# gabrielspmoreira/chameleon_recsys

Hardware: NVIDIA H100
Metric: NAR train interactions/sec (higher is better)
Workload: dtype f32 (wgmma: bf16x3 (error-compensated) forward, single-pass TF32 backward; fp32 accumulate)

## Files before the change

chameleon_recsys_b200/_lib.py:

```python
from __future__ import annotations

import ctypes as C
import os
from typing import Optional

HERE = os.path.dirname(os.path.abspath(__file__))
LIB_PATH = os.path.join(HERE, 'libnar_b200.so')

NAR_MAX_SEGMENTS = 24
NAR_MAX_SRC = 16
NAR_MAX_COLS = 1024

ACT_NONE, ACT_LEAKY, ACT_TANH = 0, 1, 2


class NarError(RuntimeError):
    pass


class Segment(C.Structure):
    _fields_ = [('kind', C.c_int32), ('col', C.c_int32), ('width', C.c_int32), ('card', C.c_int32),
                ('src', C.c_int32), ('ld', C.c_int32), ('table', C.c_void_p), ('grad', C.c_void_p)]


# ... 41 lines not shown
class StepIO(C.Structure):
    _fields_ = [('B', C.c_int64), ('Bg', C.c_int64), ('T', C.c_int64), ('sess0', C.c_int64), ('L', C.c_int64),
                ('L_global', C.c_int64), ('L_cap', C.c_int64), ('global_step', C.c_int64),
                ('sampler_step', C.c_uint32), ('train', C.c_int32),
                ('all_items', C.c_void_p), ('event_ts', C.c_void_p), ('item_clicked', C.c_void_p), ('label_next', C.c_void_p),
                ('buffer', C.c_void_p), ('max_ts', C.c_void_p), ('pop_norm', C.c_void_p),
                ('ctx_int', C.c_void_p * NAR_MAX_SRC), ('ctx_float', C.c_void_p * NAR_MAX_SRC),
                ('pos_idx', C.c_void_p), ('sess_off', C.c_void_p),
                ('prep_ws', C.c_void_p), ('prep_ws_bytes', C.c_int64), ('ws', C.c_void_p), ('ws_bytes', C.c_int64),
                ('loss', C.c_void_p)]


class NoveltyReg(C.Structure):
    _fields_ = [('factor', C.c_float), ('log_base', C.c_float), ('pop_norm', C.c_void_p), ('cand_ids', C.c_void_p),
                ('loss_nov', C.c_void_p)]


class GemmEpilogue(C.Structure):
    _fields_ = [('bias', C.c_void_p), ('act', C.c_int32), ('dact', C.c_int32), ('aux', C.c_void_p),
                ('ld_aux', C.c_int64), ('accumulate', C.c_int32), ('split_k', C.c_int32),
                ('precision', C.c_int32), ('b_lo', C.c_void_p), ('b_bf16', C.c_void_p), ('ld_bf16', C.c_int64),
                ('a_scale', C.c_void_p), ('ld_a_scale', C.c_int64), ('a_scale_group', C.c_int64),
                ('pred', C.c_void_p), ('d_pred', C.c_void_p), ('ld_pred', C.c_int64), ('pred_group', C.c_int64),
                ('car_pp', C.c_void_p), ('car_pc', C.c_void_p), ('car_pi', C.c_void_p), ('car_pos_idx', C.c_void_p),
                ('car_neg_uidx', C.c_void_p), ('car_dpp', C.c_void_p), ('car_dpc', C.c_void_p), ('car_dpi', C.c_void_p),
                ('ld_car', C.c_int64), ('car_k', C.c_int64)]


_lib: Optional[C.CDLL] = None

i64, i32, f32, vp, u64, u32 = C.c_int64, C.c_int32, C.c_float, C.c_void_p, C.c_uint64, C.c_uint32

_SIGNATURES = {
    'nar_abi_version': (C.c_int, []),
    'nar_abi_struct_size': (C.c_int, [C.c_int]),
    'nar_status_string': (C.c_char_p, [C.c_int]),
    'nar_ctx_create': (C.c_int, [C.c_int, C.POINTER(vp)]),
    'nar_ctx_destroy': (C.c_int, [vp]),
    'nar_gather_features': (C.c_int, [vp, C.POINTER(FeaturePlanC), vp, vp, C.POINTER(RowLayout), vp, vp, vp, vp]),
    'nar_gather_features_bwd': (C.c_int, [vp, C.POINTER(FeaturePlanC), vp, vp, C.POINTER(RowLayout), vp, vp, vp, vp, vp, vp]),
    'nar_build_base_rows': (C.c_int, [vp, i64, vp, vp, vp, vp, i64, vp, i64, vp, vp, vp]),
    'nar_sample_negatives_uidx': (C.c_int, [vp, vp, i64, i64, i64, i64, vp, i64, i64, i64, u64, u32, vp, vp,
                                            C.POINTER(vp), C.POINTER(vp), vp, i64, vp]),
    'nar_car_combine': (C.c_int, [vp, vp, vp, vp, vp, i64, i64, i64, C.c_int, vp, vp]),
    'nar_car_combine_t': (C.c_int, [vp, vp, vp, vp, vp, i64, i64, i64, C.c_int, vp, i64, vp]),
    'nar_engine_create': (C.c_int, [vp, C.POINTER(ModelCfg), C.POINTER(vp)]),
    'nar_engine_destroy': (C.c_int, [vp]),
# ... 114 lines not shown
```

chameleon_recsys_b200/csrc/engine.cu:

```cuda
#include "common.cuh"
#include <string.h>
#include <stdio.h>
#include <stdlib.h>

extern "C" int nar_sample_negatives_uidx(nar_ctx*, const int64_t*, int64_t, int64_t, int64_t, int64_t, const int64_t*, int64_t,
                                         int64_t, int64_t, uint64_t, uint32_t, int64_t*, int32_t*, const int64_t**,
                                         const int32_t**, void*, int64_t, void*);
namespace nar {
int recommend_rows(const int32_t* pos_idx, int64_t L, const int64_t* item_clicked, const int64_t* cand_ids, int64_t N,
                   int32_t* row_pos, int64_t* row_item, cudaStream_t st);
}

namespace {

constexpr int N_EVENTS = 64;

inline int64_t align_up(int64_t x, int64_t a) { return (x + a - 1) / a * a; }

struct Carver {
  char* base; int64_t off;
  explicit Carver(void* b) : base(static_cast<char*>(b)), off(0) {}
  template <typename T> T* take(int64_t n) {
    T* p = base ? reinterpret_cast<T*>(base + off) : nullptr;
    off = align_up(off + (n > 0 ? n : 1) * (int64_t)sizeof(T), 256);
// ... 178 lines not shown
    chk(nar_gemm_tf32(e->ctx, M, N, Kd, X, ldx, x_kmajor, W(off_W), ldw, 0, Y, ldy, &ep, st));
  }
  void dgrad(const float* dY, int64_t lddy, int64_t off_W, int64_t ldw, float* dX, int64_t lddx, int64_t M, int64_t n_in,
             int64_t n_out, int dact, const float* auxp, int64_t ld_aux, int accumulate, cudaStream_t st) {
    nar_gemm_epilogue ep; memset(&ep, 0, sizeof(ep));
    ep.dact = dact; ep.aux = auxp; ep.ld_aux = ld_aux; ep.accumulate = accumulate; ep.split_k = accumulate ? 0 : 1;
    ep.precision = c.bwd_precision;
    chk(nar_gemm_tf32(e->ctx, M, n_in, n_out, dY, lddy, 1, W(off_W), ldw, 1, dX, lddx, &ep, st));
  }
  void wgrad(const float* X, int64_t ldx, const float* dY, int64_t lddy, int64_t off_W, int64_t ldw, int64_t n_in, int64_t n_out,
             int64_t rows, cudaStream_t st, const float* a_scale = nullptr, int64_t ld_scale = 0, int64_t group = 0) {
    nar_gemm_epilogue ep; memset(&ep, 0, sizeof(ep));
    ep.a_scale = a_scale; ep.ld_a_scale = ld_scale; ep.a_scale_group = group;
    ep.accumulate = 1; ep.split_k = 0; ep.precision = c.bwd_precision;
    chk(nar_gemm_tf32(e->ctx, n_in, n_out, rows, X, ldx, 0, dY, lddy, 0, G(off_W), ldw, &ep, st));
  }
  void wgrad_xt(const float* XT, int64_t ldxt, const float* dY, int64_t lddy, int64_t off_W, int64_t ldw, int64_t n_in,
                int64_t n_out, int64_t rows, cudaStream_t st) {
    nar_gemm_epilogue ep; memset(&ep, 0, sizeof(ep));
    ep.accumulate = 1; ep.split_k = 0; ep.precision = c.bwd_precision;
    chk(nar_gemm_tf32_dt(e->ctx, n_out, n_in, rows, dY, lddy, 0, XT, ldxt, 1, G(off_W), ldw, &ep, st));
  }
  void dgrad_prod(const float* dY, int64_t lddy, int64_t off_W, int64_t ldw, const float* cand, const float* pred, int64_t group,
                  float* dX, float* dpred, int64_t M, int64_t n_in, int64_t n_out, cudaStream_t st) {
    nar_gemm_epilogue ep; memset(&ep, 0, sizeof(ep));
    ep.dact = NAR_ACT_TANH; ep.aux = cand; ep.ld_aux = n_in; ep.split_k = 1; ep.precision = c.bwd_precision;
    ep.pred = pred; ep.d_pred = dpred; ep.ld_pred = n_in; ep.pred_group = group;
    chk(nar_gemm_tf32(e->ctx, M, n_in, n_out, dY, lddy, 1, W(off_W), ldw, 1, dX, n_in, &ep, st));
  }
  void dgrad_car(const float* dY, int64_t lddy, int64_t off_W, int64_t ldw, const float* PP, const float* PC, const float* PI,
                 const int32_t* pos_idx, const int32_t* neg_uidx, float* dPP, float* dPC, float* dPI, int64_t M, int64_t n_in,
                 int64_t n_out, cudaStream_t st) {
    nar_gemm_epilogue ep; memset(&ep, 0, sizeof(ep));
    ep.dact = NAR_ACT_LEAKY_RELU; ep.split_k = 1; ep.precision = c.bwd_precision;
    ep.car_pp = PP; ep.car_pc = PC; ep.car_pi = PI; ep.car_pos_idx = pos_idx; ep.car_neg_uidx = neg_uidx;
    ep.car_dpp = dPP; ep.car_dpc = dPC; ep.car_dpi = dPI; ep.ld_car = n_in; ep.car_k = c.K;
    chk(nar_gemm_tf32(e->ctx, M, n_in, n_out, dY, lddy, 1, W(off_W), ldw, 1, nullptr, 0, &ep, st));
  }
  void bgrad(const float* dY, int64_t ld, int64_t rows, int64_t cols, int64_t off_b, cudaStream_t st) {
    chk(nar_colsum_add(dY, rows, cols, ld, G(off_b), st));
  }
  void dropout(const float* src, float* dst, int64_t rows, int64_t cols, const int32_t* row_pos, int tensor_id, cudaStream_t st) {
    chk(nar_dropout_rows(src, dst, rows, cols, cols, row_pos, io->L, c.K + 1, c.K, tensor_id, c.keep_prob, c.dropout_seed,
                         (uint32_t)(io->global_step + 1), st));
  }
  void scorer(const float* Ec, const float* PR, int64_t n_pos, int64_t n_cand, bool fused, float* PD, float* Z1, float* Z2,
              float* Z3, float* logits, float* loss, float inv_count, float* dZ3, float* dE, float* dPR,
              const nar_novelty_reg* nov) {
    const int64_t R = n_pos * n_cand, C = c.C;
    if (c.ranking == 0) {
// ... 84 lines not shown
  nar_novelty_reg nov; memset(&nov, 0, sizeof(nov));
  nov.factor = c.novelty_reg_factor; nov.log_base = c.plan.log_base_novelty; nov.pop_norm = io->pop_norm;
  nov.cand_ids = pb.row_item + L; nov.loss_nov = io->loss + 2;
  const nar_novelty_reg* novp = c.novelty_reg_factor > 0.f ? &nov : nullptr;
  const bool fused = fused_product(e);
  s.scorer(Ec, sb.PR, L, n_cand, fused, sb.PD, sb.Z1, sb.Z2, sb.Z3, sb.logits, io->loss, inv_count, train ? sb.dZ3 : nullptr,
           train ? sb.dE + L * C : nullptr, train ? sb.dPR : nullptr, novp);
  if (c.reg_l2 > 0.f && c.rank == 0) { cudaStream_t st = s.fork(); s.chk(nar_l2_loss_add(c.params, c.reg_end, c.reg_l2, io->loss + 1, st)); }
  if (!train || s.rc) { s.join(); return s.rc; }

  float* dEc = sb.dE + L * C;
  if (c.ranking == 0) {
    { cudaStream_t st = s.fork(); s.wgrad(sb.Z2, 64, sb.dZ3, 32, c.off_M[2], c.ld_M[2], 64, 32, Rc, st); s.bgrad(sb.dZ3, 32, Rc, 32, c.off_c[2], st); }
    s.dgrad(sb.dZ3, 32, c.off_M[2], c.ld_M[2], sb.dZ2, 64, Rc, 64, 32, NAR_ACT_LEAKY_RELU, sb.Z2, 64, 0, main);
    { cudaStream_t st = s.fork(); s.wgrad(sb.Z1, 128, sb.dZ2, 64, c.off_M[1], c.ld_M[1], 128, 64, Rc, st); s.bgrad(sb.dZ2, 64, Rc, 64, c.off_c[1], st); }
    s.dgrad(sb.dZ2, 64, c.off_M[1], c.ld_M[1], sb.dZ1, 128, Rc, 128, 64, NAR_ACT_LEAKY_RELU, sb.Z1, 128, 0, main);
    {
      cudaStream_t st = s.fork();
      if (fused) s.wgrad(Ec, C, sb.dZ1, 128, c.off_M[0], c.ld_M[0], C, 128, Rc, st, sb.PR, C, n_cand);
      else s.wgrad(sb.PD, C, sb.dZ1, 128, c.off_M[0], c.ld_M[0], C, 128, Rc, st);
      s.bgrad(sb.dZ1, 128, Rc, 128, c.off_c[0], st);
    }
    if (fused) {
      s.dgrad_prod(sb.dZ1, 128, c.off_M[0], c.ld_M[0], Ec, sb.PR, n_cand, dEc, sb.dPR, Rc, C, 128, main);
    } else {
      s.dgrad(sb.dZ1, 128, c.off_M[0], c.ld_M[0], sb.dPD, C, Rc, C, 128, NAR_ACT_NONE, nullptr, 0, 0, main);
      s.chk(nar_mul_pred_bwd(sb.dPD, Ec, sb.PR, L, n_cand, C, NAR_ACT_TANH, dEc, sb.dPR, main));
    }
  } else {
    s.chk(nar_act_bwd(dEc, Ec, Rc * C, NAR_ACT_TANH, dEc, main));
  }
  {
    cudaStream_t st = s.fork();
    if (c.dedup) s.wgrad_xt(sb.H1cT, sb.ldr, dEc, C, c.off_W2, C, C, C, Rc, st);
    else s.wgrad(H1c, C, dEc, C, c.off_W2, C, C, C, Rc, st);
    s.bgrad(dEc, C, Rc, C, c.off_b2, st);
  }
  {
    s.chk(nar_act_bwd(sb.dPR, sb.PR, L * C, NAR_ACT_TANH, sb.dPR, main));
    { cudaStream_t st = s.fork(); s.wgrad(sb.F1, 512, sb.dPR, C, c.off_W4, C, 512, C, L, st); s.bgrad(sb.dPR, C, L, C, c.off_b4, st); }
    s.dgrad(sb.dPR, C, c.off_W4, C, sb.dF1, 512, L, 512, C, NAR_ACT_LEAKY_RELU, sb.F1, 512, 0, main);
    if (drop) s.dropout(sb.dF1, sb.dF1, L, 512, io->pos_idx, 4, main);
    const float* rnn_out = drop ? sb.HOd[c.layers - 1] : sb.HO[c.layers - 1];
    { cudaStream_t st = s.fork(); s.wgrad(rnn_out, Hp, sb.dF1, 512, c.off_W3, 512, Hp, 512, L, st); s.bgrad(sb.dF1, 512, L, 512, c.off_b3, st); }
    s.dgrad(sb.dF1, 512, c.off_W3, 512, sb.dHO, Hp, L, Hp, 512, NAR_ACT_NONE, nullptr, 0, 0, main);
    float* dho = sb.dHO;
    for (int i = c.layers - 1; i >= 0; --i) {
      if (drop) s.dropout(dho, dho, L, Hp, io->pos_idx, 8 + i, main);
      const float* x_in = i == 0 ? sb.E : (drop ? sb.HOd[i - 1] : sb.HO[i - 1]);
      const int64_t n_in = i == 0 ? C : Hp;
      const int64_t gw = gate_blocks(c) * Hp;
      if (c.rnn_cell == NAR_CELL_GRU) {
        float* cand_T = e->WhT[i] + 2 * Hp * Hp;
        s.chk(nar_transpose_f32(s.W(c.off_Wh[i]), Hp, 2 * Hp, 2 * Hp, e->WhT[i], Hp, main));
        s.chk(nar_transpose_f32(s.W(c.off_Whc[i]), Hp, Hp, Hp, cand_T, Hp, main));
        s.chk(nar_gru_bwd(e->ctx, dho, sb.HO[i], sb.GT[i], sb.UO[i], sb.CD[i], e->WhT[i], cand_T, io->sess_off, B, Hp, sb.dGX[i],
                          sb.HPV[i], main));
      } else {
        s.chk(nar_transpose_f32(s.W(c.off_Wh[i]), Hp, gw, gw, e->WhT[i], Hp, main));
// ... 327 lines not shown
                                    void* stream) {
  if (!e || !io || !io->ws || !q_pos || !cand_ids || !out_ids || !io->buffer || !io->pop_norm || !io->item_clicked) return NAR_ERR_INVALID;
  if (io->train) return NAR_ERR_INVALID;
  return run_recommend(e, io, q_rows, q_pos, Q, cand_ids, N, top_n, exclude_session_clicks, q_block, n_block, out_ids, out_scores,
                       out_probs, as_stream(stream));
}

extern "C" int64_t nar_engine_launch_count(const nar_engine* e) { return e ? e->launches : 0; }

extern "C" int nar_engine_buffer(const nar_engine* e, const nar_step_io* io, const char* name, void** ptr, int64_t* rows, int64_t* ld) {
  if (!e || !io || !name || !ptr) return NAR_ERR_INVALID;
  const nar_model_cfg& c = e->cfg;
  const int64_t L = io->L, K = c.K, n_cand = K + 1, Rc = L * n_cand, R = L + Rc;
  PrepBufs pb; StepBufs sb;
  prep_carve(e, io->Bg, io->B, io->T, io->L_cap, io->prep_ws, &pb);
  step_carve(e, io->L_cap, io->train, io->ws, &sb);
  const int64_t NB = 2 * L + pb.U;
  struct Ent { const char* n; void* p; int64_t r, l; };
  const Ent tab[] = {
      {"neg", pb.neg, io->Bg * io->T, K}, {"neg_uidx", pb.neg_uidx, io->Bg * io->T, K}, {"stats", pb.stats, 1, 24},
      {"row_pos", pb.row_pos, R, 1}, {"row_item", pb.row_item, R, 1}, {"base_pos", pb.base_pos, NB, 1},
      {"base_item", pb.base_item, NB, 1},
      {"X", sb.X, c.dedup ? NB : R, c.Fp}, {"dX", sb.dX, c.dedup ? NB : R, c.Fp}, {"H1", sb.H1, R, c.C}, {"H1cT", sb.H1cT, c.C, sb.ldr}, {"E", sb.E, R, c.C},
      {"dE", sb.dE, R, c.C}, {"dH1", sb.dH1, R, c.C}, {"F1", sb.F1, L, 512}, {"PR", sb.PR, L, c.C},
      {"logits", sb.logits, L, n_cand}, {"PD", sb.PD, Rc, c.C}, {"Z1", sb.Z1, Rc, 128}, {"Z2", sb.Z2, Rc, 64}, {"Z3", sb.Z3, Rc, 32}, {"PP", sb.PP, L, c.C},
      {"PI", sb.PI, pb.U, c.C}, {"PC", sb.PC, L, c.C}, {"DB", sb.DB, 3 * L + pb.U, c.C},
      {"HO0", sb.HO[0], L, c.Hp}, {"HO1", sb.HO[1], L, c.Hp}, {"HO2", sb.HO[2], L, c.Hp}, {"HO3", sb.HO[3], L, c.Hp},
      {"HOd0", sb.HOd[0], L, c.Hp}, {"HOd1", sb.HOd[1], L, c.Hp}, {"HOd2", sb.HOd[2], L, c.Hp}, {"HOd3", sb.HOd[3], L, c.Hp}};
  for (const Ent& t : tab)
    if (strcmp(t.n, name) == 0) {
      *ptr = t.p;
      if (rows) *rows = t.r;
      if (ld) *ld = t.l;
      return t.p ? NAR_OK : NAR_ERR_INVALID;
    }
  return NAR_ERR_INVALID;
}
```

chameleon_recsys_b200/csrc/gemm_wgmma.cu:

```cuda
#include "common.cuh"
#include <cuda_bf16.h>
#include <stdlib.h>
#include <string.h>
#include <type_traits>

namespace nar {
namespace gemm {

constexpr int BM = 128;
constexpr int BN = 128;
constexpr int BK = 32;
constexpr int TILE_BYTES = 128 * BK * 4;
constexpr int NUM_THREADS = 256;
constexpr int EPI_LD = BN + 4;

constexpr int EXT_SCALE_SMEM = 1, EXT_SCALE_GMEM = 2, EXT_PROD_BWD = 3, EXT_CAR_BWD = 4, EXT_TRANS_D = 5;
constexpr int SC_ROWS_K = 32, SC_ROWS_MN = 8;
constexpr int SC_BYTES = 4096;
static_assert(SC_ROWS_K * BK * 4 == SC_BYTES && SC_ROWS_MN * BM * 4 == SC_BYTES, "a_scale slice per stage");

template <int MODE, bool B_MN, int SC = 0> struct Cfg {
  static constexpr bool SPLIT3 = MODE == 1 || MODE == 2;
  static constexpr bool BLO = MODE == 2;
  static constexpr bool PREP = B_MN || SPLIT3;
  static constexpr bool PREP_TILES = SPLIT3;
  static constexpr int STAGE_BYTES = TILE_BYTES * (BLO ? 3 : 2);
  static constexpr int CTAS_PER_SM = PREP_TILES ? 1 : 2;
  static constexpr int STAGES = (BLO || !PREP_TILES) ? 3 : 4;
  static constexpr int PREP_TILE_BYTES = PREP_TILES ? TILE_BYTES * 2 : 0;
  static constexpr int PREP_BYTES = 2 * PREP_TILE_BYTES;
  static constexpr int SC_OFF = STAGES * STAGE_BYTES + PREP_BYTES;
  static constexpr int BAR_OFF = SC_OFF + STAGES * SC;
  static constexpr int SMEM_BYTES = BAR_OFF + 64 + 1024;
  static_assert(STAGES * STAGE_BYTES >= BM * EPI_LD * 4, "the epilogue stages the accumulators in the operand ring");
  static_assert(SMEM_BYTES <= 227 * 1024, "227 KB of shared memory per block");
  static_assert(CTAS_PER_SM * (SMEM_BYTES + 1024) <= 228 * 1024, "228 KB of shared memory per SM (1 KB reserved per block)");
};

struct Params {
  int64_t M, N, K;
  float* D; int64_t ldd;
  const float* bias;
  const float* aux; int64_t ld_aux;
  int act, dact, accumulate;
  int k_tiles_per_split;
  int n_tiles;
  const float* a_scale; int64_t ld_a_scale, a_rows, a_cols; uint32_t group;
  const float* pred; float* d_pred; int64_t ld_pred, n_pos; int pos_per_tile;
  const float *car_pp, *car_pc, *car_pi; const int32_t *car_pos_idx, *car_neg_uidx;
  float *car_dpp, *car_dpc, *car_dpi; int64_t ld_car; int car_k;
};

__device__ __forceinline__ uint32_t smem_u32(const void* p) { return (uint32_t)__cvta_generic_to_shared(p); }

__device__ __forceinline__ void mbar_init(uint64_t* bar, uint32_t count) {
  asm volatile("mbarrier.init.shared::cta.b64 [%0], %1;" ::"r"(smem_u32(bar)), "r"(count) : "memory");
}
__device__ __forceinline__ void mbar_expect_tx(uint64_t* bar, uint32_t bytes) {
  asm volatile("mbarrier.arrive.expect_tx.shared::cta.b64 _, [%0], %1;" ::"r"(smem_u32(bar)), "r"(bytes) : "memory");
}
__device__ __forceinline__ void mbar_wait(uint64_t* bar, uint32_t parity) {
  const uint32_t addr = smem_u32(bar);
  uint32_t ok = 0;
  for (uint32_t it = 0; it < (1u << 26); ++it) {
    asm volatile(
        "{\n\t.reg .pred p;\n\t"
        "mbarrier.try_wait.parity.shared::cta.b64 p, [%1], %2;\n\t"
        "selp.u32 %0, 1, 0, p;\n\t}"
        : "=r"(ok) : "r"(addr), "r"(parity) : "memory");
    if (ok) return;
  }
// ... 171 lines not shown
#pragma unroll 1
  for (int c = tid; c < TILE_BYTES / 16; c += NUM_THREADS) {
    int row, col;
    if (A_MN) { const int kr = (c >> 3) & 31; row = k_elem + kr; col = m0 + (c >> 8) * 32 + (((c & 7) ^ (kr & 7)) << 2); }
    else { const int r = c >> 3; row = m0 + r; col = k_elem + (((c & 7) ^ (r & 7)) << 2); }
    float4* x = reinterpret_cast<float4*>(sa + c * 16);
    float4 v = *x;
    v.x = __fmul_rn(v.x, scale_gmem(p, row, col)); v.y = __fmul_rn(v.y, scale_gmem(p, row, col + 1));
    v.z = __fmul_rn(v.z, scale_gmem(p, row, col + 2)); v.w = __fmul_rn(v.w, scale_gmem(p, row, col + 3));
    *x = v;
  }
}
__device__ __forceinline__ float2 ld_shared_f2(uint32_t addr) {
  float2 v;
  asm volatile("ld.shared.v2.f32 {%0, %1}, [%2];" : "=f"(v.x), "=f"(v.y) : "r"(addr));
  return v;
}
__device__ __forceinline__ float ld_shared_f32(uint32_t addr) {
  float v;
  asm volatile("ld.shared.f32 %0, [%1];" : "=f"(v) : "r"(addr));
  return v;
}

__device__ __forceinline__ void prod_bwd_epilogue(const Params& p, const float* stage, int m_blk, int n_blk, int tid) {
  const int P = p.pos_per_tile, g = (int)p.group;
  for (int idx = tid; idx < P * BN; idx += NUM_THREADS) {
    const int pl = idx / BN, c = idx % BN;
    const int64_t pos = (int64_t)m_blk * P + pl, col = (int64_t)n_blk * BN + c;
    if (pos >= p.n_pos || col >= p.N) continue;
    const float pr = __ldg(p.pred + pos * p.ld_pred + col);
    const float* v = stage + pl * g * EPI_LD + c;
    const float* e = p.aux + pos * g * p.ld_aux + col;
    float* d = p.D + pos * g * p.ldd + col;
    float acc = 0.f;
    int j = 0;
    for (; j + 8 <= g; j += 8) {
      float ev[8];
#pragma unroll
      for (int u = 0; u < 8; ++u) ev[u] = e[(j + u) * p.ld_aux];
#pragma unroll
      for (int u = 0; u < 8; ++u) {
        const float x = v[(j + u) * EPI_LD];
        d[(j + u) * p.ldd] = x * pr * act_grad_from_output(ev[u], p.dact);
        acc = fmaf(x, ev[u], acc);
      }
    }
    for (; j < g; ++j) {
      const float x = v[j * EPI_LD], ej = e[j * p.ld_aux];
      d[j * p.ldd] = x * pr * act_grad_from_output(ej, p.dact);
      acc = fmaf(x, ej, acc);
    }
    p.d_pred[pos * p.ld_pred + col] = acc;
  }
}

__device__ __forceinline__ void car_bwd_row(const Params& p, int m0, int tid, int32_t& l, int32_t& u) {
  l = -1; u = -1;
  const int row = m0 + tid, n_cand = p.car_k + 1;
  if (tid >= BM || row >= p.M) return;
  l = row / n_cand;
  const int j = row - l * n_cand;
  if (j > 0) u = __ldg(p.car_neg_uidx + (int64_t)__ldg(p.car_pos_idx + l) * p.car_k + j - 1);
}

__device__ __forceinline__ void car_bwd_epilogue(const Params& p, float* stage, const int32_t* s_l, const int32_t* s_u, int m0,
                                                 int n_blk, int tid) {
  constexpr int RB = 8;
  const int warp = tid >> 5, c4 = (tid & 31) * 4;
  const int64_t col = (int64_t)n_blk * BN + c4;
  const int64_t ld = p.ld_car;
  if (col < p.N) {
#pragma unroll 1
    for (int it0 = 0; it0 < BM / 8; it0 += RB) {
      float4 a[RB], b[RB];
#pragma unroll
// ... 247 lines not shown
    if (kt < num_kt) k_tile(kt, std::integral_constant<int, 0>());
  }
  wgmma_wait<0>();
  fence_acc(acc);
  __syncthreads();

  float* stage = reinterpret_cast<float*>(smem);
  int32_t* s_l = reinterpret_cast<int32_t*>(stage + BM * EPI_LD);
  int32_t* s_u = s_l + BM;
  if (CAR_BWD && tid < BM) { s_l[tid] = car_l; s_u[tid] = car_u; }
#pragma unroll
  for (int j = 0; j < 16; ++j) {
    const int c = 8 * j + 2 * t;
    if (TRANS_D) {
      stage[c * EPI_LD + r0] = acc[4 * j]; stage[(c + 1) * EPI_LD + r0] = acc[4 * j + 1];
      stage[c * EPI_LD + r0 + 8] = acc[4 * j + 2]; stage[(c + 1) * EPI_LD + r0 + 8] = acc[4 * j + 3];
    } else {
      *reinterpret_cast<float2*>(stage + r0 * EPI_LD + c) = make_float2(acc[4 * j], acc[4 * j + 1]);
      *reinterpret_cast<float2*>(stage + (r0 + 8) * EPI_LD + c) = make_float2(acc[4 * j + 2], acc[4 * j + 3]);
    }
  }
  __syncthreads();
  if (PROD_BWD) {
    prod_bwd_epilogue(p, stage, m_blk, n_blk, tid);
    return;
  }
  if (CAR_BWD) {
    car_bwd_epilogue(p, stage, s_l, s_u, m0, n_blk, tid);
    return;
  }
  if (TRANS_D) {
    const int64_t col = (int64_t)m0 + lane * 4;
    if (col >= p.M) return;
    for (int it = 0; it < BN / 8; ++it) {
      const int nl = it * 8 + warp;
      const int64_t row = (int64_t)n_blk * BN + nl;
      if (row >= p.N) break;
      const float4 v = *reinterpret_cast<const float4*>(stage + nl * EPI_LD + lane * 4);
      float* d = p.D + row * p.ldd + col;
      if (col + 4 <= p.M) {
        if (p.accumulate) atomicAdd(reinterpret_cast<float4*>(d), v);
        else *reinterpret_cast<float4*>(d) = v;
      } else {
        const float e[4] = {v.x, v.y, v.z, v.w};
#pragma unroll
        for (int j = 0; j < 3; ++j)
          if (col + j < p.M) { if (p.accumulate) atomicAdd(d + j, e[j]); else d[j] = e[j]; }
// ... 148 lines not shown
  auto is_act = [](int32_t a) { return a == NAR_ACT_NONE || a == NAR_ACT_LEAKY_RELU || a == NAR_ACT_TANH; };
  if (!is_act(epi->act) || !is_act(epi->dact)) return NAR_ERR_INVALID;
  if (epi->split_k > 1 && (epi->bias || epi->act)) return NAR_ERR_INVALID;
  const bool bf16 = epi->precision == 4;
  if (bf16 && (!epi->b_bf16 || epi->accumulate || epi->split_k > 1)) return NAR_ERR_INVALID;
  const bool blo = epi->precision == 3 && epi->b_lo != nullptr;
  const int mode = bf16 ? 4 : (epi->precision == 1 ? 0 : (blo ? 2 : 1));
  const bool scale = epi->a_scale != nullptr, prod_bwd = epi->pred != nullptr;
  const int64_t a_rows = a_kmajor ? M : K, a_cols = a_kmajor ? K : M;
  if (trans_d && ((mode != 0 && mode != 1) || a_kmajor || !b_kmajor || epi->bias || epi->act || epi->dact || epi->aux || scale ||
                  prod_bwd || car_bwd)) return NAR_ERR_INVALID;
  if (scale) {
    if (!((mode == 4 && a_kmajor) || (mode == 0 && !a_kmajor && !b_kmajor)) || prod_bwd) return NAR_ERR_INVALID;
    if (epi->a_scale_group < 1 || a_rows > 0x7fffffffLL || a_cols > 0x7fffffffLL || epi->a_scale_group > a_rows ||
        epi->ld_a_scale < a_cols || (epi->ld_a_scale & 3) != 0 ||
        (reinterpret_cast<uintptr_t>(epi->a_scale) & 15u) != 0) return NAR_ERR_INVALID;
  } else if (epi->a_scale_group != 0 || epi->ld_a_scale != 0) {
    return NAR_ERR_INVALID;
  }
  if (prod_bwd) {
    const int64_t g = epi->pred_group;
    if (mode != 0 || !a_kmajor || !b_kmajor || epi->accumulate || epi->split_k > 1 || epi->bias || epi->act) return NAR_ERR_INVALID;
    if (g < 1 || g > BM || M % g != 0 || !epi->d_pred || !epi->aux || epi->ld_aux < N || epi->ld_pred < N) return NAR_ERR_INVALID;
  } else if (epi->d_pred || epi->pred_group != 0 || epi->ld_pred != 0) {
    return NAR_ERR_INVALID;
  }
  if (car_bwd) {
    const int64_t kk = epi->car_k, ld = epi->ld_car;
    auto al16 = [](const void* q) { return q && (reinterpret_cast<uintptr_t>(q) & 15u) == 0; };
    if ((mode != 0 && mode != 1) || !a_kmajor || !b_kmajor || epi->accumulate || epi->split_k > 1 || epi->bias || epi->act ||
        epi->aux || scale || prod_bwd) return NAR_ERR_INVALID;
    if (kk < 1 || kk > 0x7fffffffLL - 1 || M > 0x7fffffffLL - BM || M % (kk + 1) != 0 || (N & 3) != 0 || ld < N || (ld & 3) != 0)
      return NAR_ERR_INVALID;
    if (!al16(epi->car_pp) || !al16(epi->car_pc) || !al16(epi->car_pi) || !al16(epi->car_dpp) || !al16(epi->car_dpc) ||
        !al16(epi->car_dpi) || !epi->car_pos_idx || !epi->car_neg_uidx) return NAR_ERR_INVALID;
  } else if (epi->car_pc || epi->car_pi || epi->car_pos_idx || epi->car_neg_uidx || epi->car_dpp || epi->car_dpc || epi->car_dpi ||
             epi->ld_car != 0 || epi->car_k != 0) {
    return NAR_ERR_INVALID;
  }
  const int64_t pos_per_tile = prod_bwd ? BM / epi->pred_group : 0, n_pos = prod_bwd ? M / epi->pred_group : 0;
  const int64_t n_tiles = (N + BN - 1) / BN, m_tiles = prod_bwd ? (n_pos + pos_per_tile - 1) / pos_per_tile : (M + BM - 1) / BM;
  if (n_tiles * m_tiles > 0x7fffffffLL) return NAR_ERR_UNSUPPORTED;
  const int k_tiles = (int)((K + BK - 1) / BK);
  const bool amn = !a_kmajor, bmn = !b_kmajor;
  int split = epi->split_k;
  if (split <= 0) {
    split = 1;
// ... 6 lines not shown
    }
  }
  if (split > k_tiles) split = k_tiles;
  if (split > 1 && !epi->accumulate) return NAR_ERR_INVALID;
  int per = (k_tiles + split - 1) / split;
  split = (k_tiles + per - 1) / per;
  CUtensorMap ta, tb;
  int rc = make_operand_map(ctx, &ta, A, M, K, lda, a_kmajor != 0);
  if (rc) return rc;
  if (bf16) rc = make_bf16_plane_map(ctx, &tb, epi->b_bf16, N, k_tiles, epi->ld_bf16);
  else rc = make_operand_map(ctx, &tb, B, N, K, ldb, b_kmajor != 0);
  if (rc) return rc;
  CUtensorMap tbl = tb;
  if (blo) {
    rc = make_operand_map(ctx, &tbl, epi->b_lo, N, K, ldb, b_kmajor != 0);
    if (rc) return rc;
  }
  Params p;
  p.M = M; p.N = N; p.K = K; p.D = D; p.ldd = ldd; p.bias = epi->bias; p.aux = epi->aux; p.ld_aux = epi->ld_aux;
  p.act = epi->act; p.dact = epi->dact; p.accumulate = epi->accumulate; p.k_tiles_per_split = per;
  p.n_tiles = (int)n_tiles;
  p.a_scale = epi->a_scale; p.ld_a_scale = epi->ld_a_scale; p.a_rows = a_rows; p.a_cols = a_cols;
  p.group = (uint32_t)(scale ? epi->a_scale_group : (prod_bwd ? epi->pred_group : 1));
  p.pred = epi->pred; p.d_pred = epi->d_pred; p.ld_pred = epi->ld_pred; p.n_pos = n_pos; p.pos_per_tile = (int)pos_per_tile;
  p.car_pp = epi->car_pp; p.car_pc = epi->car_pc; p.car_pi = epi->car_pi; p.car_pos_idx = epi->car_pos_idx;
  p.car_neg_uidx = epi->car_neg_uidx; p.car_dpp = epi->car_dpp; p.car_dpc = epi->car_dpc; p.car_dpi = epi->car_dpi;
  p.ld_car = epi->ld_car; p.car_k = (int)epi->car_k;
  dim3 grid((unsigned)(n_tiles * m_tiles), (unsigned)split, 1);
  cudaStream_t st = as_stream(stream);
  if (scale) {
    const int64_t span = (a_kmajor ? BM - 1 : BK - 1) / epi->a_scale_group + 2;
    if (span <= (a_kmajor ? SC_ROWS_K : SC_ROWS_MN)) {
      rc = make_scale_map(ctx, &tbl, epi->a_scale, (a_rows + epi->a_scale_group - 1) / epi->a_scale_group, a_cols, epi->ld_a_scale,
                          !a_kmajor);
      if (rc) return rc;
      if (mode == 4) return launch<false, false, 4, EXT_SCALE_SMEM>(ta, tb, tbl, p, grid, st);
      return launch<true, true, 0, EXT_SCALE_SMEM>(ta, tb, tbl, p, grid, st);
    }
    if (mode == 4) return launch<false, false, 4, EXT_SCALE_GMEM>(ta, tb, tbl, p, grid, st);
    return launch<true, true, 0, EXT_SCALE_GMEM>(ta, tb, tbl, p, grid, st);
  }
  if (prod_bwd) return launch<false, false, 0, EXT_PROD_BWD>(ta, tb, tbl, p, grid, st);
  if (car_bwd) {
    if (mode == 0) return launch<false, false, 0, EXT_CAR_BWD>(ta, tb, tbl, p, grid, st);
    return launch<false, false, 1, EXT_CAR_BWD>(ta, tb, tbl, p, grid, st);
  }
  if (trans_d) {
// ... 30 lines not shown
```

chameleon_recsys_b200/ops.py:

```python
from __future__ import annotations

import ctypes as C
from typing import Optional

import torch

from . import _lib
from ._lib import ACT_LEAKY, ACT_NONE, ACT_TANH, Context, FeaturePlanC, GemmEpilogue, NarError, check

_ctx: dict = {}
LAUNCHES = 0


def context(device: Optional[int] = None) -> Context:
    if device is None:
        device = torch.cuda.current_device()
    if device not in _ctx:
        _ctx[device] = Context(device)
    return _ctx[device]


_STREAM_OVERRIDE: Optional[int] = None


# ... 13 lines not shown
        _STREAM_OVERRIDE = self.prev
        return False


def _stream() -> C.c_void_p:
    if _STREAM_OVERRIDE is not None:
        return C.c_void_p(_STREAM_OVERRIDE)
    return C.c_void_p(torch.cuda.current_stream().cuda_stream)


def _p(t: Optional[torch.Tensor]) -> C.c_void_p:
    return C.c_void_p(0 if t is None else t.data_ptr())


def _chk_f32(*ts):
    for t in ts:
        if t is not None:
            assert t.is_cuda and t.dtype == torch.float32, (t.device, t.dtype)


def gemm(A: torch.Tensor, B: torch.Tensor, D: torch.Tensor, M: int, N: int, K: int, *, a_kmajor=True, b_kmajor=True,
         lda=None, ldb=None, ldd=None, bias=None, act=ACT_NONE, dact=ACT_NONE, aux=None, ld_aux=None,
         accumulate=False, split_k=1, precision=3, b_lo=None, b_bf16=None, ld_bf16=0, a_scale=None, a_scale_group=0,
         pred=None, d_pred=None, pred_group=0, car=None, trans_d=False):
    global LAUNCHES
    LAUNCHES += 1
    """D[M,N] = epilogue(sum_k A(m,k) B(n,k)); see nar_gemm_tf32.  a_scale / pred / d_pred: row strides from the tensors.
    car: dict(pp, pc, pi, pos_idx, neg_uidx, dpp, dpc, dpi, k) for the CAR layer-1 backward epilogue (D = None; ld_car from
    pp).  trans_d: D stored transposed, D[n*ldd + m] (nar_gemm_tf32_dt)."""
    _chk_f32(A, B, D, bias, aux, a_scale, pred, d_pred)
    lda = A.stride(0) if lda is None else lda
    ldb = (B.stride(0) if B is not None else 0) if ldb is None else ldb
    ldd = (D.stride(0) if D is not None else 0) if ldd is None else ldd
    epi = GemmEpilogue(_p(bias), act, dact, _p(aux), (aux.stride(0) if (aux is not None and ld_aux is None) else (ld_aux or 0)),
                       1 if accumulate else 0, int(split_k), int(precision), _p(b_lo), _p(b_bf16), int(ld_bf16),
                       _p(a_scale), a_scale.stride(0) if a_scale is not None else 0, int(a_scale_group),
                       _p(pred), _p(d_pred), pred.stride(0) if pred is not None else 0, int(pred_group))
    if car is not None:
        _chk_f32(car['pp'], car['pc'], car['pi'], car['dpp'], car['dpc'], car['dpi'])
        assert car['pos_idx'].dtype == torch.int32 and car['neg_uidx'].dtype == torch.int32
        for f in ('pp', 'pc', 'pi', 'pos_idx', 'neg_uidx', 'dpp', 'dpc', 'dpi'):
            setattr(epi, 'car_' + f, _p(car[f]))
        epi.ld_car, epi.car_k = car['pp'].stride(0), int(car['k'])
    ctx = context()
    fn = 'nar_gemm_tf32_dt' if trans_d else 'nar_gemm_tf32'
    check(getattr(ctx.lib, fn)(ctx.handle, M, N, K, _p(A), lda, 1 if a_kmajor else 0, _p(B), ldb, 1 if b_kmajor else 0,
                               _p(D), ldd, C.byref(epi), _stream()), fn)


_PACK_SCRATCH: dict = {}


def pack_bf16x3(W: torch.Tensor, K: int, N: int) -> torch.Tensor:
    global LAUNCHES
    LAUNCHES += 1
    ld_out = (K + 31) // 32 * 64
    out = torch.zeros(N, ld_out, dtype=torch.bfloat16, device=W.device)
    dev = W.device.index
    if dev not in _PACK_SCRATCH:
        _PACK_SCRATCH[dev] = torch.zeros(32 * 32, dtype=torch.uint8, device=W.device)
# ... 235 lines not shown
```

include/nar_b200.h:

```cpp
#ifndef NAR_B200_H
#define NAR_B200_H

#include <stdint.h>

#ifdef __cplusplus
extern "C" {
#endif

#define NAR_ABI_VERSION 3

typedef enum {
  NAR_OK = 0,
  NAR_ERR_INVALID = -1,
  NAR_ERR_UNSUPPORTED = -2,
  NAR_ERR_NO_DEVICE = -3,
  NAR_ERR_WORKSPACE = -4
} nar_status;

typedef struct nar_ctx nar_ctx;

int  nar_abi_version(void);
int  nar_abi_struct_size(int which);
const char* nar_status_string(int status);
int  nar_ctx_create(int device, nar_ctx** out);
// ... 76 lines not shown

typedef enum { NAR_ACT_NONE = 0, NAR_ACT_LEAKY_RELU = 1, NAR_ACT_TANH = 2 } nar_act;
typedef enum { NAR_CELL_UGRNN = 0, NAR_CELL_GRU = 1, NAR_CELL_LSTM = 2 } nar_rnn_cell;

typedef struct {
  const float* bias;
  int32_t act;
  int32_t dact;
  const float* aux;
  int64_t ld_aux;
  int32_t accumulate;
  int32_t split_k;
  int32_t precision;
  const float* b_lo;
  const void* b_bf16;
  int64_t ld_bf16;
  const float* a_scale;
  int64_t ld_a_scale;
  int64_t a_scale_group;
  const float* pred;
  float* d_pred;
  int64_t ld_pred;
  int64_t pred_group;
  const float* car_pp;
  const float* car_pc;
  const float* car_pi;
  const int32_t* car_pos_idx;
  const int32_t* car_neg_uidx;
  float* car_dpp;
  float* car_dpc;
  float* car_dpi;
  int64_t ld_car;
  int64_t car_k;
} nar_gemm_epilogue;

int nar_pack_bf16x3(const float* const* W , void* const* out , const int32_t* K, const int32_t* N,
                    const int32_t* ldw, const int32_t* ld_out, int n, void* descs_dev, void* stream);

int nar_gemm_tf32(nar_ctx* ctx, int64_t M, int64_t N, int64_t K,
                  const float* A, int64_t lda, int a_kmajor,
                  const float* B, int64_t ldb, int b_kmajor,
                  float* D, int64_t ldd, const nar_gemm_epilogue* epi , void* stream);
int nar_gemm_tf32_dt(nar_ctx* ctx, int64_t M, int64_t N, int64_t K,
                     const float* A, int64_t lda, int a_kmajor,
                     const float* B, int64_t ldb, int b_kmajor,
                     float* D, int64_t ldd, const nar_gemm_epilogue* epi , void* stream);
// ... 206 lines not shown
```

Baseline: 301,600.

## Fuse b2 bias gradient into product-backward GEMM epilogue and vectorize it

The prod-backward epilogue is restructured so each warp processes rows with float4 loads and stores, staging the Ec rows in shared memory for the d_pred reductions. It also accumulates per-column sums of the output and atomically adds them into a new d_bias field. This removes the separate bgrad kernel for b2 when the fused path is used. The cost is extra shared-memory staging, more syncthreads, and atomics in the epilogue, plus an ABI struct change.

```diff
diff --git a/chameleon_recsys_b200/_lib.py b/chameleon_recsys_b200/_lib.py
--- a/chameleon_recsys_b200/_lib.py
+++ b/chameleon_recsys_b200/_lib.py
@@ -87,7 +87,7 @@
                 ('precision', C.c_int32), ('b_lo', C.c_void_p), ('b_bf16', C.c_void_p), ('ld_bf16', C.c_int64),
                 ('a_scale', C.c_void_p), ('ld_a_scale', C.c_int64), ('a_scale_group', C.c_int64),
                 ('pred', C.c_void_p), ('d_pred', C.c_void_p), ('ld_pred', C.c_int64), ('pred_group', C.c_int64),
-                ('car_pp', C.c_void_p), ('car_pc', C.c_void_p), ('car_pi', C.c_void_p), ('car_pos_idx', C.c_void_p),
+                ('d_bias', C.c_void_p), ('car_pp', C.c_void_p), ('car_pc', C.c_void_p), ('car_pi', C.c_void_p), ('car_pos_idx', C.c_void_p),
                 ('car_neg_uidx', C.c_void_p), ('car_dpp', C.c_void_p), ('car_dpc', C.c_void_p), ('car_dpi', C.c_void_p),
                 ('ld_car', C.c_int64), ('car_k', C.c_int64)]
 
diff --git a/chameleon_recsys_b200/csrc/engine.cu b/chameleon_recsys_b200/csrc/engine.cu
--- a/chameleon_recsys_b200/csrc/engine.cu
+++ b/chameleon_recsys_b200/csrc/engine.cu
@@ -224,10 +224,10 @@
     chk(nar_gemm_tf32_dt(e->ctx, n_out, n_in, rows, dY, lddy, 0, XT, ldxt, 1, G(off_W), ldw, &ep, st));
   }
   void dgrad_prod(const float* dY, int64_t lddy, int64_t off_W, int64_t ldw, const float* cand, const float* pred, int64_t group,
-                  float* dX, float* dpred, int64_t M, int64_t n_in, int64_t n_out, cudaStream_t st) {
+                  float* dX, float* dpred, int64_t off_b, int64_t M, int64_t n_in, int64_t n_out, cudaStream_t st) {
     nar_gemm_epilogue ep; memset(&ep, 0, sizeof(ep));
     ep.dact = NAR_ACT_TANH; ep.aux = cand; ep.ld_aux = n_in; ep.split_k = 1; ep.precision = c.bwd_precision;
-    ep.pred = pred; ep.d_pred = dpred; ep.ld_pred = n_in; ep.pred_group = group;
+    ep.pred = pred; ep.d_pred = dpred; ep.ld_pred = n_in; ep.pred_group = group; ep.d_bias = G(off_b);
     chk(nar_gemm_tf32(e->ctx, M, n_in, n_out, dY, lddy, 1, W(off_W), ldw, 1, dX, n_in, &ep, st));
   }
   void dgrad_car(const float* dY, int64_t lddy, int64_t off_W, int64_t ldw, const float* PP, const float* PC, const float* PI,
@@ -358,7 +358,7 @@
       s.bgrad(sb.dZ1, 128, Rc, 128, c.off_c[0], st);
     }
     if (fused) {
-      s.dgrad_prod(sb.dZ1, 128, c.off_M[0], c.ld_M[0], Ec, sb.PR, n_cand, dEc, sb.dPR, Rc, C, 128, main);
+      s.dgrad_prod(sb.dZ1, 128, c.off_M[0], c.ld_M[0], Ec, sb.PR, n_cand, dEc, sb.dPR, c.off_b2, Rc, C, 128, main);
     } else {
       s.dgrad(sb.dZ1, 128, c.off_M[0], c.ld_M[0], sb.dPD, C, Rc, C, 128, NAR_ACT_NONE, nullptr, 0, 0, main);
       s.chk(nar_mul_pred_bwd(sb.dPD, Ec, sb.PR, L, n_cand, C, NAR_ACT_TANH, dEc, sb.dPR, main));
@@ -370,7 +370,7 @@
     cudaStream_t st = s.fork();
     if (c.dedup) s.wgrad_xt(sb.H1cT, sb.ldr, dEc, C, c.off_W2, C, C, C, Rc, st);
     else s.wgrad(H1c, C, dEc, C, c.off_W2, C, C, C, Rc, st);
-    s.bgrad(dEc, C, Rc, C, c.off_b2, st);
+    if (!fused) s.bgrad(dEc, C, Rc, C, c.off_b2, st);
   }
   {
     s.chk(nar_act_bwd(sb.dPR, sb.PR, L * C, NAR_ACT_TANH, sb.dPR, main));
@@ -744,7 +744,7 @@
       {"row_pos", pb.row_pos, R, 1}, {"row_item", pb.row_item, R, 1}, {"base_pos", pb.base_pos, NB, 1},
       {"base_item", pb.base_item, NB, 1},
       {"X", sb.X, c.dedup ? NB : R, c.Fp}, {"dX", sb.dX, c.dedup ? NB : R, c.Fp}, {"H1", sb.H1, R, c.C}, {"H1cT", sb.H1cT, c.C, sb.ldr}, {"E", sb.E, R, c.C},
-      {"dE", sb.dE, R, c.C}, {"dH1", sb.dH1, R, c.C}, {"F1", sb.F1, L, 512}, {"PR", sb.PR, L, c.C},
+      {"dE", sb.dE, R, c.C}, {"dPR", sb.dPR, L, c.C}, {"dH1", sb.dH1, R, c.C}, {"F1", sb.F1, L, 512}, {"PR", sb.PR, L, c.C},
       {"logits", sb.logits, L, n_cand}, {"PD", sb.PD, Rc, c.C}, {"Z1", sb.Z1, Rc, 128}, {"Z2", sb.Z2, Rc, 64}, {"Z3", sb.Z3, Rc, 32}, {"PP", sb.PP, L, c.C},
       {"PI", sb.PI, pb.U, c.C}, {"PC", sb.PC, L, c.C}, {"DB", sb.DB, 3 * L + pb.U, c.C},
       {"HO0", sb.HO[0], L, c.Hp}, {"HO1", sb.HO[1], L, c.Hp}, {"HO2", sb.HO[2], L, c.Hp}, {"HO3", sb.HO[3], L, c.Hp},
diff --git a/chameleon_recsys_b200/csrc/gemm_wgmma.cu b/chameleon_recsys_b200/csrc/gemm_wgmma.cu
--- a/chameleon_recsys_b200/csrc/gemm_wgmma.cu
+++ b/chameleon_recsys_b200/csrc/gemm_wgmma.cu
@@ -46,7 +46,7 @@
   int k_tiles_per_split;
   int n_tiles;
   const float* a_scale; int64_t ld_a_scale, a_rows, a_cols; uint32_t group;
-  const float* pred; float* d_pred; int64_t ld_pred, n_pos; int pos_per_tile;
+  const float* pred; float* d_pred; float* d_bias; int64_t ld_pred, n_pos; int pos_per_tile;
   const float *car_pp, *car_pc, *car_pi; const int32_t *car_pos_idx, *car_neg_uidx;
   float *car_dpp, *car_dpc, *car_dpi; int64_t ld_car; int car_k;
 };
@@ -264,35 +264,94 @@
   return v;
 }
 
-__device__ __forceinline__ void prod_bwd_epilogue(const Params& p, const float* stage, int m_blk, int n_blk, int tid) {
-  const int P = p.pos_per_tile, g = (int)p.group;
-  for (int idx = tid; idx < P * BN; idx += NUM_THREADS) {
-    const int pl = idx / BN, c = idx % BN;
-    const int64_t pos = (int64_t)m_blk * P + pl, col = (int64_t)n_blk * BN + c;
-    if (pos >= p.n_pos || col >= p.N) continue;
-    const float pr = __ldg(p.pred + pos * p.ld_pred + col);
-    const float* v = stage + pl * g * EPI_LD + c;
-    const float* e = p.aux + pos * g * p.ld_aux + col;
-    float* d = p.D + pos * g * p.ldd + col;
-    float acc = 0.f;
-    int j = 0;
-    for (; j + 8 <= g; j += 8) {
-      float ev[8];
-#pragma unroll
-      for (int u = 0; u < 8; ++u) ev[u] = e[(j + u) * p.ld_aux];
-#pragma unroll
-      for (int u = 0; u < 8; ++u) {
-        const float x = v[(j + u) * EPI_LD];
-        d[(j + u) * p.ldd] = x * pr * act_grad_from_output(ev[u], p.dact);
-        acc = fmaf(x, ev[u], acc);
-      }
-    }
-    for (; j < g; ++j) {
-      const float x = v[j * EPI_LD], ej = e[j * p.ld_aux];
-      d[j * p.ldd] = x * pr * act_grad_from_output(ej, p.dact);
-      acc = fmaf(x, ej, acc);
-    }
-    p.d_pred[pos * p.ld_pred + col] = acc;
+__device__ __forceinline__ float4 load4(const float* q, int nc, bool v4) {
+  if (v4 && nc == 4) return *reinterpret_cast<const float4*>(q);
+  float4 v = make_float4(0.f, 0.f, 0.f, 0.f);
+  if (nc > 0) v.x = q[0];
+  if (nc > 1) v.y = q[1];
+  if (nc > 2) v.z = q[2];
+  if (nc > 3) v.w = q[3];
+  return v;
+}
+__device__ __forceinline__ void st_global_v4(float* q, const float4& v) {
+  asm volatile("st.global.v4.f32 [%0], {%1, %2, %3, %4};" ::"l"(q), "f"(v.x), "f"(v.y), "f"(v.z), "f"(v.w) : "memory");
+}
+
+template <int EC_ROWS>
+__device__ __forceinline__ void prod_bwd_epilogue(const Params& p, float* stage, int m_blk, int n_blk, int tid) {
+  constexpr int RQ = (EC_ROWS + 7) / 8;
+  static_assert(EC_ROWS >= 8, "the eight warps' column sums reuse the Ec rows");
+  const int g = (int)p.group;
+  const int64_t pos0 = (int64_t)m_blk * p.pos_per_tile, row0 = pos0 * g;
+  const int n_pos = (int)min((int64_t)p.pos_per_tile, p.n_pos - pos0);
+  const int warp = tid >> 5, c4 = (tid & 31) * 4;
+  const int64_t col = (int64_t)n_blk * BN + c4;
+  const int nc = (int)min((int64_t)4, p.N - col);
+  const bool aux_v4 = ((reinterpret_cast<uintptr_t>(p.aux) | (uintptr_t)p.ld_aux * 4) & 15) == 0;
+  const bool pred_v4 = ((reinterpret_cast<uintptr_t>(p.pred) | (uintptr_t)p.ld_pred * 4) & 15) == 0;
+  float* ec = stage + BM * EPI_LD;
+  const int pc = g <= EC_ROWS ? EC_ROWS / g : 1;
+  float4 bsum = make_float4(0.f, 0.f, 0.f, 0.f);
+  float chain = 0.f;
+  for (int pb = 0; pb < n_pos; pb += pc) {
+    const int np = min(pc, n_pos - pb), pr_end = (pb + np) * g;
+    for (int r0 = pb * g; r0 < pr_end; r0 += EC_ROWS) {
+      const int r1 = min(r0 + EC_ROWS, pr_end);
+      if (nc > 0) {
+        float4 ev[RQ], pv[RQ];
+#pragma unroll
+        for (int q = 0; q < RQ; ++q) {
+          const int r = r0 + warp + 8 * q;
+          if (r < r1) {
+            ev[q] = load4(p.aux + (row0 + r) * p.ld_aux + col, nc, aux_v4);
+            pv[q] = load4(p.pred + (pos0 + r / g) * p.ld_pred + col, nc, pred_v4);
+          }
+        }
+#pragma unroll
+        for (int q = 0; q < RQ; ++q) {
+          const int r = r0 + warp + 8 * q;
+          if (r < r1) {
+            const float4 x = *reinterpret_cast<const float4*>(stage + r * EPI_LD + c4);
+            const float4 e = ev[q], pr = pv[q];
+            const float4 d = make_float4(x.x * pr.x * act_grad_from_output(e.x, p.dact), x.y * pr.y * act_grad_from_output(e.y, p.dact),
+                                         x.z * pr.z * act_grad_from_output(e.z, p.dact), x.w * pr.w * act_grad_from_output(e.w, p.dact));
+            float* dst = p.D + (row0 + r) * p.ldd + col;
+            if (nc == 4) {
+              st_global_v4(dst, d);
+            } else {
+              dst[0] = d.x;
+              if (nc > 1) dst[1] = d.y;
+              if (nc > 2) dst[2] = d.z;
+            }
+            *reinterpret_cast<float4*>(ec + (r - r0) * BN + c4) = e;
+            bsum.x += d.x; bsum.y += d.y; bsum.z += d.z; bsum.w += d.w;
+          }
+        }
+      }
+      __syncthreads();
+      for (int idx = tid; idx < np * BN; idx += NUM_THREADS) {
+        const int pl = pb + idx / BN, c = idx % BN;
+        const int64_t colc = (int64_t)n_blk * BN + c;
+        if (colc >= p.N) continue;
+        const int beg = max(pl * g, r0), end = min((pl + 1) * g, r1);
+        float acc = beg == pl * g ? 0.f : chain;
+#pragma unroll 8
+        for (int r = beg; r < end; ++r) acc = fmaf(stage[r * EPI_LD + c], ec[(r - r0) * BN + c], acc);
+        if (end == (pl + 1) * g) p.d_pred[(pos0 + pl) * p.ld_pred + colc] = acc;
+        else chain = acc;
+      }
+      __syncthreads();
+    }
+  }
+  if (p.d_bias) {
+    float* part = ec;
+    *reinterpret_cast<float4*>(part + warp * BN + c4) = bsum;
+    __syncthreads();
+    if (tid < BN && (int64_t)n_blk * BN + tid < p.N) {
+      const float* s = part + tid;
+      const float t = ((s[0] + s[BN]) + (s[2 * BN] + s[3 * BN])) + ((s[4 * BN] + s[5 * BN]) + (s[6 * BN] + s[7 * BN]));
+      atomicAdd(p.d_bias + (int64_t)n_blk * BN + tid, t);
+    }
   }
 }
 
@@ -586,7 +645,7 @@
   }
   __syncthreads();
   if (PROD_BWD) {
-    prod_bwd_epilogue(p, stage, m_blk, n_blk, tid);
+    prod_bwd_epilogue<(C::STAGES * C::STAGE_BYTES - BM * EPI_LD * 4) / (BN * 4)>(p, stage, m_blk, n_blk, tid);
     return;
   }
   if (CAR_BWD) {
@@ -781,7 +840,7 @@
     const int64_t g = epi->pred_group;
     if (mode != 0 || !a_kmajor || !b_kmajor || epi->accumulate || epi->split_k > 1 || epi->bias || epi->act) return NAR_ERR_INVALID;
     if (g < 1 || g > BM || M % g != 0 || !epi->d_pred || !epi->aux || epi->ld_aux < N || epi->ld_pred < N) return NAR_ERR_INVALID;
-  } else if (epi->d_pred || epi->pred_group != 0 || epi->ld_pred != 0) {
+  } else if (epi->d_pred || epi->pred_group != 0 || epi->ld_pred != 0 || epi->d_bias) {
     return NAR_ERR_INVALID;
   }
   if (car_bwd) {
@@ -834,7 +893,7 @@
   p.n_tiles = (int)n_tiles;
   p.a_scale = epi->a_scale; p.ld_a_scale = epi->ld_a_scale; p.a_rows = a_rows; p.a_cols = a_cols;
   p.group = (uint32_t)(scale ? epi->a_scale_group : (prod_bwd ? epi->pred_group : 1));
-  p.pred = epi->pred; p.d_pred = epi->d_pred; p.ld_pred = epi->ld_pred; p.n_pos = n_pos; p.pos_per_tile = (int)pos_per_tile;
+  p.pred = epi->pred; p.d_pred = epi->d_pred; p.d_bias = epi->d_bias; p.ld_pred = epi->ld_pred; p.n_pos = n_pos; p.pos_per_tile = (int)pos_per_tile;
   p.car_pp = epi->car_pp; p.car_pc = epi->car_pc; p.car_pi = epi->car_pi; p.car_pos_idx = epi->car_pos_idx;
   p.car_neg_uidx = epi->car_neg_uidx; p.car_dpp = epi->car_dpp; p.car_dpc = epi->car_dpc; p.car_dpi = epi->car_dpi;
   p.ld_car = epi->ld_car; p.car_k = (int)epi->car_k;
diff --git a/chameleon_recsys_b200/ops.py b/chameleon_recsys_b200/ops.py
--- a/chameleon_recsys_b200/ops.py
+++ b/chameleon_recsys_b200/ops.py
@@ -59,20 +59,21 @@
 def gemm(A: torch.Tensor, B: torch.Tensor, D: torch.Tensor, M: int, N: int, K: int, *, a_kmajor=True, b_kmajor=True,
          lda=None, ldb=None, ldd=None, bias=None, act=ACT_NONE, dact=ACT_NONE, aux=None, ld_aux=None,
          accumulate=False, split_k=1, precision=3, b_lo=None, b_bf16=None, ld_bf16=0, a_scale=None, a_scale_group=0,
-         pred=None, d_pred=None, pred_group=0, car=None, trans_d=False):
+         pred=None, d_pred=None, pred_group=0, d_bias=None, car=None, trans_d=False):
     global LAUNCHES
     LAUNCHES += 1
     """D[M,N] = epilogue(sum_k A(m,k) B(n,k)); see nar_gemm_tf32.  a_scale / pred / d_pred: row strides from the tensors.
+    d_bias: += the column sums of D (with pred only).
     car: dict(pp, pc, pi, pos_idx, neg_uidx, dpp, dpc, dpi, k) for the CAR layer-1 backward epilogue (D = None; ld_car from
     pp).  trans_d: D stored transposed, D[n*ldd + m] (nar_gemm_tf32_dt)."""
-    _chk_f32(A, B, D, bias, aux, a_scale, pred, d_pred)
+    _chk_f32(A, B, D, bias, aux, a_scale, pred, d_pred, d_bias)
     lda = A.stride(0) if lda is None else lda
     ldb = (B.stride(0) if B is not None else 0) if ldb is None else ldb
     ldd = (D.stride(0) if D is not None else 0) if ldd is None else ldd
     epi = GemmEpilogue(_p(bias), act, dact, _p(aux), (aux.stride(0) if (aux is not None and ld_aux is None) else (ld_aux or 0)),
                        1 if accumulate else 0, int(split_k), int(precision), _p(b_lo), _p(b_bf16), int(ld_bf16),
                        _p(a_scale), a_scale.stride(0) if a_scale is not None else 0, int(a_scale_group),
-                       _p(pred), _p(d_pred), pred.stride(0) if pred is not None else 0, int(pred_group))
+                       _p(pred), _p(d_pred), pred.stride(0) if pred is not None else 0, int(pred_group), _p(d_bias))
     if car is not None:
         _chk_f32(car['pp'], car['pc'], car['pi'], car['dpp'], car['dpc'], car['dpi'])
         assert car['pos_idx'].dtype == torch.int32 and car['neg_uidx'].dtype == torch.int32
diff --git a/include/nar_b200.h b/include/nar_b200.h
--- a/include/nar_b200.h
+++ b/include/nar_b200.h
@@ -122,6 +122,7 @@
   float* d_pred;
   int64_t ld_pred;
   int64_t pred_group;
+  float* d_bias;
   const float* car_pp;
   const float* car_pc;
   const float* car_pi;
```

Result: faster. 310,700, median of 6 (+3.0%).
